# grasingerm/polymer-stats

Hardware: AMD Instinct MI355X
Metric: MC monomer-updates/sec (whole node) at n=100 (higher is better)
Workload: dtype f64

## Files before the change

polymer_stats_amd/csrc/pstat_kernels.hip:

```cpp
#include "pstat_device.h"

#include <hip/hip_runtime.h>
#include <math.h>
#include <type_traits>

#include "../../include/pstat.h"
#include "pstat_math.h"

#ifndef PSTAT_GM_DEPTH
#define PSTAT_GM_DEPTH 2
#endif
#ifndef PSTAT_GI_DEPTH
#define PSTAT_GI_DEPTH 1
#endif
#ifndef PSTAT_GI_CC
#define PSTAT_GI_CC 1
#endif
#ifndef PSTAT_UNROLL_ISING
#define PSTAT_UNROLL_ISING 16
#endif
#ifndef PSTAT_UNROLL
#define PSTAT_UNROLL 16
#endif

namespace pstat {

#ifndef PSTAT_PART

template <typename R, typename G>
__global__ void init_kernel(SweepArgs A, DevState S, const CaseConst *__restrict__ cases,
                            int chain_type, int energy_type, double phi_step, double theta_step,
                            InitOpts io) {
  int64_t c = (int64_t)blockIdx.x * blockDim.x + threadIdx.x;
  if (c >= S.C) return;
  const int64_t icase = c / A.chains_per_case, local = c % A.chains_per_case;
  const CaseConst cc = cases[icase];
  R *th = (R *)S.ang, *ph = (R *)S.ang + A.n * S.C;
  G g;
  g.seed(cc.seed, cc.chain_id0 + (uint64_t)local);
  if (io.use_x0 == 2) {
    for (int64_t i = 0; i < A.n; ++i)
      ph[i * S.C + c] = store_phi_rad<R>(io.x0_vec[2 * i] + io.dx0_phi * u01<double>(g.next()));
    for (int64_t i = 0; i < A.n; ++i)
      th[i * S.C + c] = store_theta_rad<R>(io.x0_vec[2 * i + 1] + io.dx0_theta * u01<double>(g.next()));
  } else if (io.use_x0) {
    for (int64_t i = 0; i < A.n; ++i)
      ph[i * S.C + c] = store_phi_rad<R>(io.x0_phi + io.dx0_phi * u01<double>(g.next()));
    for (int64_t i = 0; i < A.n; ++i)
      th[i * S.C + c] = store_theta_rad<R>(io.x0_theta + io.dx0_theta * u01<double>(g.next()));
  } else {
    for (int64_t i = 0; i < A.n; ++i) ph[i * S.C + c] = store_phi<R>(u01<double>(g.next()));
    for (int64_t i = 0; i < A.n; ++i) th[i * S.C + c] = store_theta<R>(u01<double>(g.next()));
  }

  double r[3] = {0, 0, 0}, p[3] = {0, 0, 0}, usum = 0, upair = 0, omega = 0, c2sum = 0, psisum = 0;
  double pnx = 0, pny = 0, pnz = 0, pmx = 0, pmy = 0, pmz = 0;
  for (int64_t i = 0; i < A.n; ++i) {
    double t = load_theta<R>(th[i * S.C + c]), f = load_phi<R>(ph[i * S.C + c]);
    double st = sin(t), ct = cos(t), sp = sin(f), cp = cos(f);
    double nx = cp * st, ny = sp * st, nz = ct, mx, my, mz;
    if (chain_type == PSTAT_DIELECTRIC)
      dipole<double, PSTAT_DIELECTRIC>((cc.K1 - cc.K2) * cc.E0, cc.K2 * cc.E0, nx, ny, nz, mx, my, mz);
    else
      dipole<double, PSTAT_POLAR>(cc.mu, 0.0, nx, ny, nz, mx, my, mz);
    r[0] += cc.b * nx; r[1] += cc.b * ny; r[2] += cc.b * nz;
    p[0] += mx; p[1] += my; p[2] += mz;
    usum += -0.5 * cc.E0 * mz;
    omega += log(st);
    c2sum += ct * ct;
    if (i > 0) {
      const double psi = acos(fmin(1.0, fmax(-1.0, pnx * nx + pny * ny + pnz * nz)));
      psisum += psi;
      usum += cc.kappa / 2 * (psi - cc.psi0) * (psi - cc.psi0);
    }
    if (energy_type == PSTAT_ISING && i > 0) {
      double h = -cc.b / 2;
      upair += pair_term<double>(h * (pnx + nx), h * (pny + ny), h * (pnz + nz), pmx, pmy, pmz, mx, my, mz);
    }
    pnx = nx; pny = ny; pnz = nz; pmx = mx; pmy = my; pmz = mz;
  }
  double U = usum + upair - (r[0] * cc.Fx + r[2] * cc.Fz);
  S.obs[OBS_R1 * S.C + c] = r[0]; S.obs[OBS_R2 * S.C + c] = r[1]; S.obs[OBS_R3 * S.C + c] = r[2];
  S.obs[OBS_P1 * S.C + c] = p[0]; S.obs[OBS_P2 * S.C + c] = p[1]; S.obs[OBS_P3 * S.C + c] = p[2];
  S.obs[OBS_U * S.C + c] = U; S.obs[OBS_USUM * S.C + c] = usum;
  S.obs[OBS_C2 * S.C + c] = c2sum; S.obs[OBS_PSI * S.C + c] = psisum;
  g.store(S.rng + c, S.C);
  S.stepsz[0 * S.C + c] = phi_step; S.stepsz[1 * S.C + c] = theta_step;
  S.win[0 * S.C + c] = 0; S.win[1 * S.C + c] = 0;
  S.nacc_total[c] = 0;
  for (int q = 0; q < NSUMS; ++q) S.sums[q * S.C + c] = 0.0;
  S.wnorm[c] = 0.0;
  S.lag[c] = 0.0;
  S.uref[c] = usum;
  S.nanrej[c] = 0;
  (void)omega;
}

#endif


struct Draw {
  uint32_t idx, cell, wphi, wth, weps, wflip;
  uint32_t w0;
};

template <typename G, bool WIDE> struct StepGen : G {};
template <> struct StepGen<Mwc64x, true> {
  uint64_t t;
  uint32_t sh;
  __device__ inline void load(const uint32_t *p, int64_t stride) {
    t = (uint64_t)p[0] | ((uint64_t)p[stride] << 32);
    sh = 32;
    asm volatile("" : "+v"(sh));
  }
  __device__ inline uint32_t next() {
    const uint32_t x = (uint32_t)t, r = x ^ (uint32_t)(t >> 32);
    t = (uint64_t)x * Mwc64x::A + (t >> sh);
    return r;
  }
  __device__ inline void store(uint32_t *p, int64_t stride) const {
    p[0] = (uint32_t)t; p[stride] = (uint32_t)(t >> 32); p[2 * stride] = 0u; p[3 * stride] = 0u;
  }
};

template <bool RARE, typename G>
__device__ __forceinline__ Draw draw_step(G &g, uint32_t n, bool flips, uint32_t row_bytes, uint32_t lane_bytes) {
  Draw d;
  d.w0 = g.next();
  d.idx = __umulhi(d.w0, n);
  d.cell = __umul24(d.idx, row_bytes) + lane_bytes;
  d.wphi = g.next();
  d.wflip = 0;
  if constexpr (RARE) {
    if (flips) d.wflip = g.next();
  }
  d.wth = g.next();
  d.weps = g.next();
  return d;
}

template <typename R, typename G, int CT, int EN, bool FX, bool RARE, int ST>
__device__ __forceinline__ void run_segment(const SweepArgs &A, const DevState &S, const CaseConst &cc,
                                            const SweepRare rare, unsigned char *smem, const int lane,
                                            const int64_t c, int64_t step, int64_t remaining, const int blk) {
  using R2 = typename Vec2<R>::type;
  using AG = Ang<R>;
  constexpr bool Q = ST == 1;
  constexpr bool GM = ST == 2;
  static_assert(!Q || sizeof(R) == 4, "the lattice state runs on f32 arithmetic");
  static_assert(!GM || sizeof(R) == 8, "global-memory state: f64");
  constexpr bool GI = GM && EN == PSTAT_ISING;
  constexpr int DEPTH = GI ? PSTAT_GI_DEPTH : PSTAT_GM_DEPTH;
  using Cell = typename std::conditional<Q, uint32_t, R2>::type;
  const int lanes = GM ? 64 : A.lanes;
  unsigned char *const cells = GM ? reinterpret_cast<unsigned char *>(S.work) + (size_t)blk * (size_t)A.n * 64 * sizeof(Cell) : smem;
  Cell *ang = reinterpret_cast<Cell *>(cells);
  const int64_t C = S.C;
  const int n = (int)A.n;

  const R Fz = (R)cc.Fz, Fx = (R)cc.Fx, b = (R)cc.b, kT = (R)cc.kT;
  const R a_or_mu = (CT == PSTAT_DIELECTRIC) ? (R)((cc.K1 - cc.K2) * cc.E0) : (R)cc.mu;
  const R k2e = (R)(cc.K2 * cc.E0);
  const R mhalfE0 = (R)(-0.5 * cc.E0);
  const R hb = (R)(-cc.b / 2);
  const R ising_scale = cc.b == 0.0 ? (R)__builtin_nan("") : (R)(0.0795774715459476679 / fabs(cc.b * cc.b * cc.b / 8));
  const R nbeta_log2e = (R)(-1.4426950408889634 / cc.kT);
  const double ninv_kT = -1.0 / cc.kT;
  (void)ninv_kT;
  (void)Fx; (void)kT; (void)hb; (void)nbeta_log2e; (void)ising_scale;

  R maxphi = 0;
  (void)maxphi;
  if constexpr (Q) {
    const uint16_t *gth = (const uint16_t *)S.ang, *gph = (const uint16_t *)S.ang + (int64_t)n * C;
#pragma unroll 8
    for (int i = 0; i < n; ++i)
      ang[i * lanes + lane] = (uint32_t)gth[(int64_t)i * C + c] | ((uint32_t)gph[(int64_t)i * C + c] << 16);
  } else {
    const R *gth = (const R *)S.ang, *gph = (const R *)S.ang + (int64_t)n * C;
#pragma unroll 8
    for (int i = 0; i < n; ++i) {
      R2 v;
      v.x = gth[(int64_t)i * C + c];
      v.y = gph[(int64_t)i * C + c];
      if constexpr (sizeof(R) == 8) maxphi = fmax(maxphi, fabs(v.y));
      if (GM && i < A.lds_rows) reinterpret_cast<Cell *>(smem)[i * lanes + lane] = v;
      else if constexpr (GM) *reinterpret_cast<Cell *>(cells + ((EN == PSTAT_ISING && PSTAT_GI_CC) ? (uint32_t)lane * (uint32_t)n * (uint32_t)sizeof(Cell) + (uint32_t)i * (uint32_t)sizeof(Cell)
                                                                                                          : (uint32_t)(i * lanes + lane) * (uint32_t)sizeof(Cell))) = v;
      else ang[i * lanes + lane] = v;
    }
  }
  constexpr double th_unit = Q ? 3.14159265358979323846 / 65536.0 : AG::unit;
  constexpr double ph_unit = Q ? 6.28318530717958647692 / 65536.0 : AG::unit;
  StepGen<G, GM> g;
  g.load(S.rng + c, C);
  double phistep_d = S.stepsz[0 * C + c], thstep_d = S.stepsz[1 * C + c];
  R phistep = (R)(phistep_d / ph_unit), thstep = (R)(thstep_d / th_unit);
  int64_t nacc_off = S.win[0 * C + c], natt_off = S.win[1 * C + c];
  int nacc_seg = 0, steps_seg = 0;
  int nnan_seg = 0;
  R O[8];
  O[0] = (R)S.obs[OBS_R1 * C + c]; O[1] = (R)S.obs[OBS_R2 * C + c]; O[2] = (R)S.obs[OBS_R3 * C + c];
  O[3] = (R)S.obs[OBS_P1 * C + c]; O[4] = (R)S.obs[OBS_P2 * C + c]; O[5] = (R)S.obs[OBS_P3 * C + c];
  O[6] = (R)S.obs[OBS_U * C + c]; O[7] = 0;
  R usum = (R)S.obs[OBS_USUM * C + c];
  R lag = RARE ? (R)S.lag[c] : (R)0;
  const bool umb = RARE && rare.umb;
  const R wscale = umb ? (R)((0.2 + 0.8 * exp(-(cc.Fx * cc.Fx + cc.Fz * cc.Fz) / cc.kT)) / cc.kT) : (R)0;
  R uref = umb ? (R)S.uref[c] : (R)0;
  bool regauged = false;
  double wnorm = umb ? S.wnorm[c] : 0.0;
  double sums[NSUMS_BASE];
#pragma unroll
  for (int q = 0; q < NSUMS_BASE; ++q) sums[q] = S.sums[q * C + c];

  const int64_t spa = A.steps_per_adjust;
  int64_t to_adj = A.adaptive ? spa - (step % spa) : 0;
  constexpr int FLUSH = 128;
  const bool flips = RARE && rare.flips;

  using P = typename V2<R>::type;
  const uint32_t row_bytes = (uint32_t)lanes * (uint32_t)sizeof(Cell), lane_bytes = (uint32_t)lane * (uint32_t)sizeof(Cell);
  auto slot = [&](uint32_t off) __attribute__((always_inline)) -> Cell & { return *reinterpret_cast<Cell *>(cells + off); };
  constexpr bool CC = GI && PSTAT_GI_CC;
  const uint32_t chain_g = (uint32_t)lane * (uint32_t)n * (uint32_t)sizeof(Cell);
  auto gofs = [&](const uint32_t idx) __attribute__((always_inline)) -> uint32_t {
    return CC ? chain_g + idx * (uint32_t)sizeof(Cell) : idx * row_bytes + lane_bytes;
  };
  typedef int v4i __attribute__((ext_vector_type(4)));
  struct RowG { Cell l; v4i g; };
  struct RowG3 { RowG c, lo, hi; };
  using Row = typename std::conditional<GI, RowG3, typename std::conditional<GM, RowG, Cell>::type>::type;
  constexpr bool AS = GM && !CC;
  constexpr uint32_t NOWHERE = 0xFFFFFFFFu;
  const uint32_t nL = GM ? (uint32_t)A.lds_rows : 0u;
  const uint32_t trash = nL * row_bytes + lane_bytes;
  const uint32_t gbase = AS ? nL * row_bytes : 0u;
  __amdgpu_buffer_rsrc_t rsrc = __builtin_amdgcn_make_buffer_rsrc(GM ? (void *)(cells + gbase) : (void *)nullptr, 0,
                                                                  GM ? (int)((uint32_t)n * row_bytes - gbase) : 0, 0x00020000);
  auto rdcell = [&](const uint32_t idx, const uint32_t cell) __attribute__((always_inline)) -> RowG {
    RowG r;
    if constexpr (AS) {
      r.l = *reinterpret_cast<Cell *>(smem + (cell < trash ? cell : trash));
      r.g = __builtin_amdgcn_raw_buffer_load_b128(rsrc, cell - gbase, 0, 0);
    } else {
      const bool inL = idx < nL;
      r.l = *reinterpret_cast<Cell *>(smem + (inL ? cell : trash));
      r.g = __builtin_amdgcn_raw_buffer_load_b128(rsrc, inL ? 0xFFFFFFFFu : gofs(idx), 0, 0);
    }
    return r;
  };
  auto resolve = [&](const RowG &r, const uint32_t idx, const uint32_t cell, const Cell &f1, const uint32_t at1,
                     const Cell &f2, const uint32_t at2, const Cell &f3, const uint32_t at3) __attribute__((always_inline)) -> Cell {
    if constexpr (GM) {
      typedef double v2dd __attribute__((ext_vector_type(2)));
      const v2dd gv = __builtin_bit_cast(v2dd, r.g);
      const bool inL = idx < nL;
      Cell a;
      a.x = inL ? r.l.x : gv.x; a.y = inL ? r.l.y : gv.y;
      if constexpr (DEPTH == 3) {
        const bool s3 = at3 == cell;
        a.x = s3 ? f3.x : a.x; a.y = s3 ? f3.y : a.y;
      }
      if constexpr (DEPTH >= 2) {
        const bool s2 = at2 == cell;
        a.x = s2 ? f2.x : a.x; a.y = s2 ? f2.y : a.y;
      }
      const bool s1 = at1 == cell;
      a.x = s1 ? f1.x : a.x; a.y = s1 ? f1.y : a.y;
      return a;
    } else {
      return r.l;
    }
  };
  auto rdrow = [&](const Draw &d) __attribute__((always_inline)) -> Row {
    if constexpr (GI) {
      const bool hasLo = d.idx > 0, hasHi = d.idx + 1 < (uint32_t)n;
      RowG3 r;
      r.c = rdcell(d.idx, d.cell);
      r.lo = rdcell(hasLo ? d.idx - 1 : d.idx, hasLo ? d.cell - row_bytes : d.cell);
      r.hi = rdcell(hasHi ? d.idx + 1 : d.idx, hasHi ? d.cell + row_bytes : d.cell);
      return r;
    } else if constexpr (GM) {
      return rdcell(d.idx, d.cell);
    } else {
      return slot(d.cell);
    }
  };
  auto wr = [&](const Draw &d, const Cell v, const bool ok) __attribute__((always_inline)) {
    if constexpr (AS) {
      const uint32_t at = ok ? d.cell : NOWHERE;
      *reinterpret_cast<Cell *>(smem + (at < trash ? at : trash)) = v;
      typedef double v2dd __attribute__((ext_vector_type(2)));
      const v2dd vv = {v.x, v.y};
      __builtin_amdgcn_raw_buffer_store_b128(__builtin_bit_cast(v4i, vv), rsrc, at - gbase, 0, 0);
    } else if constexpr (GM) {
      const bool inL = d.idx < nL;
      *reinterpret_cast<Cell *>(smem + ((ok && inL) ? d.cell : trash)) = v;
      typedef double v2dd __attribute__((ext_vector_type(2)));
      const v2dd vv = {v.x, v.y};
      __builtin_amdgcn_raw_buffer_store_b128(__builtin_bit_cast(v4i, vv), rsrc, (ok && !inL) ? gofs(d.idx) : 0xFFFFFFFFu, 0, 0);
    } else {
      slot(d.cell) = v;
    }
  };
  Draw dA = draw_step<RARE>(g, (uint32_t)n, flips, row_bytes, lane_bytes), dB = dA;
  Row aA = rdrow(dA), aB = aA;
  Draw dC = dA;
  Row aC = aA;
  Draw dD = dA;
  Row aD = aA;
  Cell fw1_cell{}, fw2_cell{}, fw3_cell{};
  uint32_t fw1_at = ~0u, fw2_at = ~0u, fw3_at = ~0u;
  (void)dC; (void)aC; (void)dD; (void)aD; (void)fw1_cell; (void)fw2_cell; (void)fw3_cell; (void)fw1_at; (void)fw2_at; (void)fw3_at;
  if constexpr (GM && DEPTH >= 2) {
    if (remaining > 1) {
      dB = draw_step<RARE>(g, (uint32_t)n, flips, row_bytes, lane_bytes);
      aB = rdrow(dB);
    }
    if constexpr (DEPTH == 3) {
      if (remaining > 2) {
        dC = draw_step<RARE>(g, (uint32_t)n, flips, row_bytes, lane_bytes);
        aC = rdrow(dC);
      }
    }
  }
  R phistep3 = 3 * phistep, thstep3 = 3 * thstep;
  (void)phistep3; (void)thstep3;
  P stepv = {thstep, phistep}, step3v = {thstep3, phistep3};
  (void)stepv; (void)step3v;
  int left = (int)remaining;
  P Orxy = {O[0], O[1]}, Opxy = {O[3], O[4]};
  P Oz = {O[2], O[5]};
  R OU = O[6];
  const P bb = {b, b};
  (void)bb;

  auto refresh_totals = [&]() {
    double tx = 0, ty = 0, tz = 0, qx = 0, qy = 0, qz = 0, tu = 0, tp = 0;
    R pnx = 0, pny = 0, pnz = 0, pmx = 0, pmy = 0, pmz = 0;
#pragma unroll 1
    for (int i = 0; i < n; ++i) {
      const Cell a = ang[i * lanes + lane];
      R thi, phi;
      if constexpr (Q) { thi = q16_theta_turns(a & 0xFFFFu); phi = q16_phi_turns(a >> 16); }
      else { thi = a.x; phi = a.y; }
      R si, ci, spi, cpi, mix, miy, miz;
      AG::sc(thi, &si, &ci);
      AG::sc(phi, &spi, &cpi);
      const R nix = cpi * si, niy = spi * si, niz = ci;
      dipole<R, CT>(a_or_mu, k2e, nix, niy, niz, mix, miy, miz);
      tx += (double)nix; ty += (double)niy; tz += (double)niz;
      qx += (double)mix; qy += (double)miy; qz += (double)miz;
      tu += (double)(mhalfE0 * miz);
      if constexpr (EN == PSTAT_ISING) {
        if (i > 0)
          tp += (double)pair_term_fast(hb * (pnx + nix), hb * (pny + niy), hb * (pnz + niz), pmx, pmy, pmz, mix, miy, miz);
        pnx = nix; pny = niy; pnz = niz; pmx = mix; pmy = miy; pmz = miz;
      }
    }
    auto opaque = [](R v) __attribute__((always_inline)) -> R { asm volatile("" : "+v"(v)); return v; };
    const double bd = (double)b;
    Orxy.x = opaque((R)tx); Orxy.y = opaque((R)ty); Oz.x = opaque((R)tz);
    Opxy.x = opaque((R)qx); Opxy.y = opaque((R)qy); Oz.y = opaque((R)qz);
    usum = opaque((R)tu);
    OU = opaque((R)(tu + tp - ((double)Fx * bd * tx + (double)Fz * bd * tz)));
  };

  if constexpr (sizeof(R) == 4) refresh_totals();

  auto run_steps = [&](auto fold_tag) __attribute__((always_inline)) {
  constexpr bool FOLD = decltype(fold_tag)::value;
  while (left > 0) {
    int chunk = left < FLUSH ? left : FLUSH;
    if (A.adaptive && to_adj < chunk) chunk = (int)to_adj;
    P a1rxy = {0, 0}, a1pxy = {0, 0}, a2rxy = {0, 0}, a2pxy = {0, 0};
    P a1z = {0, 0}, a2z = {0, 0};
    R a1U = 0, a2U = 0;
    R accw = 0;

    auto one_step = [&](const Draw &d, const Row &a0_, Draw &dn, Row &an, const bool more)
        __attribute__((always_inline)) {
      Cell a0, aLo{}, aHi{};
      (void)aLo; (void)aHi;
      if constexpr (GI) {
        const bool hasLo = d.idx > 0, hasHi = d.idx + 1 < (uint32_t)n;
        a0 = resolve(a0_.c, d.idx, d.cell, fw1_cell, fw1_at, fw2_cell, fw2_at, fw3_cell, fw3_at);
        aLo = resolve(a0_.lo, hasLo ? d.idx - 1 : d.idx, hasLo ? d.cell - row_bytes : d.cell, fw1_cell, fw1_at, fw2_cell, fw2_at, fw3_cell, fw3_at);
        aHi = resolve(a0_.hi, hasHi ? d.idx + 1 : d.idx, hasHi ? d.cell + row_bytes : d.cell, fw1_cell, fw1_at, fw2_cell, fw2_at, fw3_cell, fw3_at);
      } else if constexpr (GM) {
        a0 = resolve(a0_, d.idx, d.cell, fw1_cell, fw1_at, fw2_cell, fw2_at, fw3_cell, fw3_at);
      } else {
        a0 = a0_;
      }
      if (more) {
        dn = draw_step<RARE>(g, (uint32_t)n, flips, row_bytes, lane_bytes);
        an = rdrow(dn);
        __builtin_amdgcn_sched_barrier(0);
      }
      R eps;
      if constexpr (sizeof(R) == 8) eps = 0;
      else eps = bits12(d.weps);
      (void)eps;
      R th0, ph0, th1, ph1;
      bool inside = true;
      uint32_t cell1 = 0;
      if constexpr (Q) {
        uint32_t k0 = a0 & 0xFFFFu;
        const uint32_t j0 = a0 >> 16;
        th0 = q16_theta_turns(k0);
        ph0 = q16_phi_turns(j0);
        if constexpr (RARE) {
          if (flips && (d.wflip >> 31)) k0 = 65535u - k0;
        }
        const int k1 = (int)k0 + q16_disp(thstep, sym11<R>(d.wth));
        const uint32_t j1 = (j0 + (uint32_t)q16_disp(phistep, sym11<R>(d.wphi))) & 0xFFFFu;
        inside = (uint32_t)k1 < 65536u;
        const uint32_t k1c = (uint32_t)min(max(k1, 0), 65535);
        th1 = q16_theta_turns(k1c);
        ph1 = q16_phi_turns(j1);
        cell1 = k1c | (j1 << 16);
      } else {
        th0 = a0.x; ph0 = a0.y;
        R flip = 0;
        if constexpr (RARE) {
          if (flips && (d.wflip >> 31)) flip = AG::theta_max - 2 * th0;
        }
        if constexpr (sizeof(R) == 8) {
          auto rounded = [](R v) __attribute__((always_inline)) -> R { asm volatile("" : "+v"(v)); return v; };
          const R dphi = rounded(phistep * rounded(sym11<R>(d.wphi)));
          R dth = rounded(thstep * rounded(sym11<R>(d.wth)));
          if constexpr (RARE) dth = rounded(flip + dth);
          ph1 = AG::wrap(ph0 + dphi);
          th1 = fmin(AG::theta_max, fmax((R)0, th0 + dth));
        } else {
          R base = th0;
          if constexpr (RARE) base = th0 + flip;
          const P basev = {base, ph0}, fv = {bits24(d.wth), bits24(d.wphi)};
          const P raw = pfma(stepv, fv, basev - step3v);
          th1 = fmin(AG::theta_max, fmax((R)0, raw.x));
          ph1 = AG::wrap(raw.y);
        }
      }
      R st0, ct0, sp0, cp0, st1, ct1, sp1, cp1;
      AG::sc_theta(th0, &st0, &ct0);
      AG::sc_theta(th1, &st1, &ct1);
      AG::template sc_phi<FOLD>(ph0, &sp0, &cp0);
      AG::template sc_phi<FOLD>(ph1, &sp1, &cp1);
      P dNxy, dMxy, D;
      R dpair = 0;
      if constexpr (EN == PSTAT_ISING && sizeof(R) == 4) {
        const P S01 = {st0, st1}, X01 = P{cp0, cp1} * S01, Y01 = P{sp0, sp1} * S01, C01 = {ct0, ct1};
        P MX01, MY01, MZ01;
        if constexpr (CT == PSTAT_DIELECTRIC) {
          const P q01 = C01 * P{a_or_mu, a_or_mu};
          MX01 = q01 * X01; MY01 = q01 * Y01;
          MZ01 = pfma(q01, C01, P{k2e, k2e});
        } else {
          const P mus = {a_or_mu, a_or_mu};
          MX01 = mus * X01; MY01 = mus * Y01; MZ01 = mus * C01;
        }
        dNxy = P{X01.y - X01.x, Y01.y - Y01.x};
        dMxy = P{MX01.y - MX01.x, MY01.y - MY01.x};
        D = P{C01.y - C01.x, MZ01.y - MZ01.x};
        P e01 = {0, 0};
        const P m3 = {-3.0f, -3.0f};
#pragma unroll
        for (int side = -1; side <= 1; side += 2) {
          const int j = (int)d.idx + side;
          if (j >= 0 && j < n) {
            const Cell aj = ang[j * lanes + lane];
            R thj, phj;
            if constexpr (Q) { thj = q16_theta_turns(aj & 0xFFFFu); phj = q16_phi_turns(aj >> 16); }
            else { thj = aj.x; phj = aj.y; }
            R sj, cj, spj, cpj, mjx, mjy, mjz;
            AG::sc(thj, &sj, &cj);
            AG::sc(phj, &spj, &cpj);
            const R njx = cpj * sj, njy = spj * sj, njz = cj;
            dipole<R, CT>(a_or_mu, k2e, njx, njy, njz, mjx, mjy, mjz);
            const P rx = X01 + P{njx, njx}, ry = Y01 + P{njy, njy}, rz = C01 + P{njz, njz};
            const P jx = {mjx, mjx}, jy = {mjy, mjy}, jz = {mjz, mjz};
            const P r2 = pfma(rz, rz, pfma(ry, ry, rx * rx));
            const P ir = {__builtin_amdgcn_rsqf(r2.x), __builtin_amdgcn_rsqf(r2.y)};
            const P ir2 = ir * ir;
            const P mimj = pfma(MZ01, jz, pfma(MY01, jy, MX01 * jx));
            const P mir = pfma(MZ01, rz, pfma(MY01, ry, MX01 * rx));
            const P mjr = pfma(jz, rz, pfma(jy, ry, jx * rx));
            const P num = pfma(m3 * ir2, mir * mjr, mimj);
            e01 = pfma(num, ir2 * ir, e01);
          }
        }
        dpair = (e01.y - e01.x) * ising_scale;
      } else {
        const P cs0 = {cp0, sp0}, cs1 = {cp1, sp1};
        const P s0s = {st0, st0}, s1s = {st1, st1};
        const P Nxy0 = cs0 * s0s, Nxy1 = cs1 * s1s;
        P Mxy0, Mxy1;
        R mz0, mz1;
        if constexpr (CT == PSTAT_DIELECTRIC) {
          const R q0 = a_or_mu * ct0, q1 = a_or_mu * ct1;
          const P q0s = {q0, q0}, q1s = {q1, q1};
          Mxy0 = q0s * Nxy0; Mxy1 = q1s * Nxy1;
          mz0 = q0 * ct0 + k2e; mz1 = q1 * ct1 + k2e;
        } else {
          const P mus = {a_or_mu, a_or_mu};
          Mxy0 = mus * Nxy0; Mxy1 = mus * Nxy1;
          mz0 = a_or_mu * ct0; mz1 = a_or_mu * ct1;
        }
        dNxy = Nxy1 - Nxy0; dMxy = Mxy1 - Mxy0;
        const P Z0 = {ct0, mz0}, Z1 = {ct1, mz1};
        D = Z1 - Z0;

        if constexpr (GI) {
          R e0 = 0, e1 = 0;
#pragma unroll
          for (int side = 0; side < 2; ++side) {
            const Cell aj = side ? aHi : aLo;
            const bool has = side ? d.idx + 1 < (uint32_t)n : d.idx > 0;
            R sj, cj, spj, cpj, mjx, mjy, mjz;
            AG::sc_theta(aj.x, &sj, &cj);
            AG::template sc_phi<FOLD>(aj.y, &spj, &cpj);
            const R njx = cpj * sj, njy = spj * sj, njz = cj;
            dipole<R, CT>(a_or_mu, k2e, njx, njy, njz, mjx, mjy, mjz);
            const R t0 = pair_term_fast(hb * (Nxy0.x + njx), hb * (Nxy0.y + njy), hb * (ct0 + njz),
                                        Mxy0.x, Mxy0.y, mz0, mjx, mjy, mjz);
            const R t1 = pair_term_fast(hb * (Nxy1.x + njx), hb * (Nxy1.y + njy), hb * (ct1 + njz),
                                        Mxy1.x, Mxy1.y, mz1, mjx, mjy, mjz);
            e0 += has ? t0 : (R)0; e1 += has ? t1 : (R)0;
          }
          dpair = e1 - e0;
        } else if constexpr (EN == PSTAT_ISING) {
          R e0 = 0, e1 = 0;
  #pragma unroll
          for (int side = -1; side <= 1; side += 2) {
            const int j = (int)d.idx + side;
            if (j >= 0 && j < n) {
              const Cell aj = ang[j * lanes + lane];
              R thj, phj;
              if constexpr (Q) { thj = q16_theta_turns(aj & 0xFFFFu); phj = q16_phi_turns(aj >> 16); }
              else { thj = aj.x; phj = aj.y; }
              R sj, cj, spj, cpj, mjx, mjy, mjz;
              AG::sc(thj, &sj, &cj);
              AG::sc(phj, &spj, &cpj);
              const R njx = cpj * sj, njy = spj * sj, njz = cj;
              dipole<R, CT>(a_or_mu, k2e, njx, njy, njz, mjx, mjy, mjz);
              e0 += pair_term_fast(hb * (Nxy0.x + njx), hb * (Nxy0.y + njy), hb * (ct0 + njz),
                                   Mxy0.x, Mxy0.y, mz0, mjx, mjy, mjz);
              e1 += pair_term_fast(hb * (Nxy1.x + njx), hb * (Nxy1.y + njy), hb * (ct1 + njz),
                                   Mxy1.x, Mxy1.y, mz1, mjx, mjy, mjz);
            }
          }
          dpair = e1 - e0;
        }
      }
      const R dmz = D.y;
      (void)dmz;

      const P dd = D * P{b, mhalfE0};
      const R drz = dd.x, du = dd.y;
      R dUi = du;
      if constexpr (EN == PSTAT_ISING) dUi = du + dpair;
      R dU;
      if constexpr (FX) dU = dUi - (Fx * (b * dNxy.x) + Fz * drz);
      else              dU = dUi - (Fz * drz);

      bool ok;
      R dw = 0;
      if constexpr (RARE) dw = du * wscale;
      if constexpr (sizeof(R) == 8) {
        ok = metropolis_f64(dU, kT, ninv_kT, st1, st0, dw - lag, A.wide_eps != 0, d.weps, d.w0, d.wphi, d.wth);
      } else {
        R e;
        if constexpr (RARE) e = __builtin_amdgcn_exp2f((R)1.44269504f * (dw - lag) + dU * nbeta_log2e);
        else                e = __builtin_amdgcn_exp2f(dU * nbeta_log2e);
        ok = eps * st0 < fma_r(st1, e, st0);
        if constexpr (Q) ok = ok && inside;
      }

      Cell a1;
      if constexpr (Q) a1 = ok ? cell1 : a0;
      else { a1.x = ok ? th1 : th0; a1.y = ok ? ph1 : ph0; }
      if constexpr (GM) { Cell t1; t1.x = th1; t1.y = ph1; wr(d, t1, ok); }
      else wr(d, a1, ok);
      const R m = ok ? (R)1 : (R)0;
      const P mm = {m, m};
      if constexpr (sizeof(R) == 8) {
        Orxy = pfma(mm, bb * dNxy, Orxy);
        Oz = pfma(mm, P{drz, dmz}, Oz);
      } else {
        Orxy = pfma(mm, dNxy, Orxy);
        Oz = pfma(mm, D, Oz);
      }
      Opxy = pfma(mm, dMxy, Opxy);
      if constexpr (EN == PSTAT_ISING) OU = ok ? OU + dU : OU;
      else                             OU = fma_r(m, dU, OU);
      if constexpr (RARE) {
        usum = fma_r(m, du, usum);
        lag = ok ? (R)0 : lag;
      }
      nacc_seg += ok ? 1 : 0;
      if constexpr (EN == PSTAT_ISING) nnan_seg += not_finite(dU) ? 1 : 0;
      if constexpr (GM) {
        fw3_cell = fw2_cell; fw3_at = fw2_at;
        fw2_cell = fw1_cell; fw2_at = fw1_at;
        fw1_cell.x = th1; fw1_cell.y = ph1; fw1_at = ok ? d.cell : ~0u;
      } else if (more) {
        const bool same = dn.cell == d.cell;
        if constexpr (Q) an = same ? a1 : an;
        else if constexpr (!GM) { an.x = same ? a1.x : an.x; an.y = same ? a1.y : an.y; }
      }

      if (umb) {
        bool raise;
        R wrel = umbrella_logw(usum, uref, wscale, raise);
        if constexpr (RARE) {
          if (__builtin_amdgcn_ballot_w64(raise) != 0) {
            if (raise) {
              const double f = exp_f64(-(double)wrel);
              const R fr = (R)f;
              const P ff = {fr, fr};
              a1rxy *= ff; a1pxy *= ff; a2rxy *= ff; a2pxy *= ff; a1z *= ff; a2z *= ff; a1U *= fr; a2U *= fr; accw *= fr;
#pragma unroll
              for (int q = 0; q < NSUMS_BASE; ++q) sums[q] *= f;
              wnorm *= f;
              uref = usum; regauged = true; wrel = 0;
            }
          }
        }
        const R wgt = exp_r(wrel);
        const P ww = {wgt, wgt};
        accw += wgt;
        a1rxy = pfma(ww, Orxy, a1rxy); a1pxy = pfma(ww, Opxy, a1pxy);
        a2rxy = pfma(ww * Orxy, Orxy, a2rxy); a2pxy = pfma(ww * Opxy, Opxy, a2pxy);
        a1z = pfma(ww, Oz, a1z); a1U = fma_r(wgt, OU, a1U);
        a2z = pfma(ww * Oz, Oz, a2z); a2U = fma_r(wgt * OU, OU, a2U);
      } else {
        a1rxy += Orxy; a1pxy += Opxy;
        a2rxy = pfma(Orxy, Orxy, a2rxy); a2pxy = pfma(Opxy, Opxy, a2pxy);
        a1z += Oz; a1U += OU;
        a2z = pfma(Oz, Oz, a2z); a2U = fma_r(OU, OU, a2U);
      }
    };
    int k = 0;
    constexpr int UNROLL = sizeof(R) == 8 ? 2 : (EN == PSTAT_ISING ? PSTAT_UNROLL_ISING : PSTAT_UNROLL);
    if constexpr (GM) {
      if constexpr (DEPTH == 3) {
        const int lim = chunk < left - 3 ? chunk : left - 3;
        for (; k + 4 <= lim; k += 4) {
          one_step(dA, aA, dD, aD, true);
          one_step(dB, aB, dA, aA, true);
          one_step(dC, aC, dB, aB, true);
          one_step(dD, aD, dC, aC, true);
        }
        for (; k < chunk; ++k) {
          one_step(dA, aA, dD, aD, left - k > 3);
          dA = dB; aA = aB;
          dB = dC; aB = aC;
          dC = dD; aC = aD;
        }
      } else if constexpr (DEPTH == 2) {
        const int lim = chunk < left - 2 ? chunk : left - 2;
        for (; k + 3 <= lim; k += 3) {
          one_step(dA, aA, dC, aC, true);
          one_step(dB, aB, dA, aA, true);
          one_step(dC, aC, dB, aB, true);
        }
        for (; k < chunk; ++k) {
          one_step(dA, aA, dC, aC, left - k > 2);
          dA = dB; aA = aB;
          dB = dC; aB = aC;
        }
      } else {
        const int lim = chunk < left - 1 ? chunk : left - 1;
        for (; k + 2 <= lim; k += 2) {
          one_step(dA, aA, dB, aB, true);
          one_step(dB, aB, dA, aA, true);
        }
        for (; k < chunk; ++k) {
          one_step(dA, aA, dB, aB, left - k > 1);
          dA = dB; aA = aB;
        }
      }
    } else {
    for (; k + (UNROLL - 1) < chunk; k += UNROLL) {
#pragma unroll
      for (int u = 0; u < UNROLL; u += 2) {
        one_step(dA, aA, dB, aB, true);
        one_step(dB, aB, dA, aA, u + 2 < UNROLL || left - k > UNROLL);
      }
    }
    for (; k + 1 < chunk; k += 2) {
      one_step(dA, aA, dB, aB, true);
      one_step(dB, aB, dA, aA, left - k > 2);
    }
    if (k < chunk) {
      one_step(dA, aA, dB, aB, left - k > 1);
      dA = dB; aA = aB;
    }
    }
// ... 374 lines not shown
```

polymer_stats_amd/csrc/pstat_math.h:

```cpp
#pragma once

#include <hip/hip_runtime.h>
#include <math.h>
#include <stdint.h>

#include "../../include/pstat.h"

namespace pstat {


template <typename R> struct Vec2;
template <> struct Vec2<float> { using type = float2; };
template <> struct Vec2<double> { using type = double2; };

template <typename R> struct K;
template <> struct K<double> {
  static constexpr double pi = 3.14159265358979323846;
  static constexpr double half_pi = 1.57079632679489661923;
};

__device__ __forceinline__ double exp_f64(const double x) {
  const double k = rint(x * 1.44269504088896338700e+00);
  const double hi = __builtin_fma(-k, 6.93147180369123816490e-01, x);
  const double r = __builtin_fma(-k, 1.90821492927058770002e-10, hi);
  double p = 1.60590438368216145994e-10;
  p = __builtin_fma(p, r, 2.08767569878680989792e-09);
  p = __builtin_fma(p, r, 2.50521083854417187751e-08);
  p = __builtin_fma(p, r, 2.75573192239858906526e-07);
  p = __builtin_fma(p, r, 2.75573192239858906526e-06);
  p = __builtin_fma(p, r, 2.48015873015873015873e-05);
  p = __builtin_fma(p, r, 1.98412698412698412698e-04);
  p = __builtin_fma(p, r, 1.38888888888888888889e-03);
  p = __builtin_fma(p, r, 8.33333333333333333333e-03);
  p = __builtin_fma(p, r, 4.16666666666666666667e-02);
  p = __builtin_fma(p, r, 1.66666666666666666667e-01);
  p = __builtin_fma(p, r, 5.00000000000000000000e-01);
  const double y = 1.0 + __builtin_fma(p, r * r, r);
  double v = ldexp(y, (int)k);
  v = x < -745.2 ? 0.0 : v;
  v = x > 709.8 ? __builtin_inf() : v;
  return v;
}
__device__ __forceinline__ double log_f64(const double x) {
  int e = __builtin_amdgcn_frexp_exp(x);
  double m = __builtin_amdgcn_frexp_mant(x);
  const bool small = m < 7.07106781186547524401e-01;
  m = small ? m + m : m;
  e = small ? e - 1 : e;
  const double f = m - 1.0, t = 2.0 + f;
  double rc = __builtin_amdgcn_rcp(t);
  rc = __builtin_fma(__builtin_fma(-t, rc, 1.0), rc, rc);
  rc = __builtin_fma(__builtin_fma(-t, rc, 1.0), rc, rc);
  const double s = f * rc, z = s * s, w = z * z;
  const double t1 = w * __builtin_fma(w, __builtin_fma(w, 1.531383769920937332e-01, 2.222219843214978396e-01), 3.999999999940941908e-01);
  const double t2 = z * __builtin_fma(w, __builtin_fma(w, __builtin_fma(w, 1.479819860511658591e-01, 1.818357216161805012e-01),
                                                       2.857142874366239149e-01), 6.666666666666735130e-01);
  const double R = t1 + t2, hfsq = 0.5 * f * f, dk = (double)e;
  double v = dk * 6.93147180369123816490e-01 - ((hfsq - (s * (hfsq + R) + dk * 1.90821492927058770002e-10)) - f);
  v = x == 0.0 ? -__builtin_inf() : v;
  v = x < 0.0 ? __builtin_nan("") : v;
  v = x == __builtin_inf() ? x : v;
  return v;
}

template <typename R>
__device__ __forceinline__ R umbrella_logw(const R usum, const R uref, const R wscale, bool &raise) {
  const R wrel = -(usum - uref) * wscale;
  constexpr R T = sizeof(R) == 4 ? (R)30 : (R)300;
  raise = wrel > T;
  return wrel;
}

__device__ __forceinline__ float exp_r(float x) { return __expf(x); }
__device__ __forceinline__ double exp_r(double x) { return exp_f64(x); }
__device__ __forceinline__ float log_r(float x) { return __logf(x); }
__device__ __forceinline__ double log_r(double x) { return log_f64(x); }
__device__ __forceinline__ float fma_r(float a, float b, float c) { return __builtin_fmaf(a, b, c); }
__device__ __forceinline__ double fma_r(double a, double b, double c) { return a * b + c; }

template <typename R>
__device__ __forceinline__ R u01(uint32_t w) {
  if constexpr (sizeof(R) == 4) return __uint_as_float(0x3F800000u | (w >> 9)) - 1.0f;
  else return (R)(w >> 9) * (R)(1.0 / 8388608.0);
}
__device__ __forceinline__ float bits12(uint32_t w) { return __uint_as_float(__builtin_amdgcn_alignbit(0x7Fu, w, 9)); }
__device__ __forceinline__ float bits24(uint32_t w) { return __uint_as_float(__builtin_amdgcn_alignbit(0x80u, w, 9)); }
template <typename R>
__device__ __forceinline__ R sym11(uint32_t w) {
  if constexpr (sizeof(R) == 4) return __uint_as_float(0x40000000u | (w >> 9)) - 3.0f;
  else return __builtin_fma((R)(w >> 9), (R)(1.0 / 4194304.0), (R)-1);
}

__device__ __forceinline__ double eps_uniform(const bool wide, const uint32_t weps, const uint32_t w0, const uint32_t wphi,
                                              const uint32_t wth) {
  const uint32_t lo = ((wth & 511u) << 12) | ((wphi & 511u) << 3) | (w0 & 7u);
  const double e53 = __builtin_fma((double)weps, 2097152.0, (double)lo) * 0x1p-53;
  const double e23 = (double)(weps >> 9) * (1.0 / 8388608.0);
#ifdef PSTAT_NARROW_EPS
  return e23;
#else
  return wide ? e53 : e23;
#endif
}

template <typename Literal>
__device__ __forceinline__ bool metropolis_filter(const double x, const double num, const double den, const uint32_t weps,
                                                  Literal &&literal) {
  const float t = (float)x;
  const float e = __builtin_amdgcn_exp2f(t * 1.44269504f);
  const float fden = (float)den;
  const float lhs = (__uint_as_float(0x3F800000u | (weps >> 9)) - 1.0f) * fden, rhs = e * (float)num;
  const float lhs_hi = __builtin_fmaf(0x1p-23f, fden, lhs);
  const float m = 2e-6f + 1e-6f * __builtin_fabsf(t);
#ifdef PSTAT_NARROW_EPS
  const bool acc = __builtin_fmaf(lhs, m, lhs) < rhs, rej = lhs > __builtin_fmaf(rhs, m, rhs);
  (void)lhs_hi;
#else
  const bool acc = __builtin_fmaf(lhs_hi, m, lhs_hi) < rhs, rej = lhs > __builtin_fmaf(rhs, m, rhs);
#endif
  bool ok = acc;
  if (__builtin_amdgcn_ballot_w64(!(acc || rej)) != 0) {
    const bool lit = literal();
    ok = (acc || rej) ? acc : lit;
  }
  return ok;
}
__device__ __forceinline__ bool metropolis_f64(const double dU, const double kT, const double ninv_kT, const double st1,
                                               const double st0, const double extra, const bool wide, const uint32_t weps,
                                               const uint32_t w0, const uint32_t wphi, const uint32_t wth) {
  return metropolis_filter(dU * ninv_kT + extra, st1, st0, weps, [&]() -> bool {
    const double delta = -dU / kT + log_f64(st1 / st0) + extra;
    const double eps = eps_uniform(wide, weps, w0, wphi, wth);
    return (delta >= 0) || (eps < exp_f64(delta));
  });
}

template <typename R, int CT>
__device__ __forceinline__ void dipole(R a_or_mu, R k2e, R nx, R ny, R nz, R &mx, R &my, R &mz) {
  if constexpr (CT == PSTAT_DIELECTRIC) {
    R a = a_or_mu * nz;
    mx = a * nx; my = a * ny; mz = a * nz + k2e;
  } else {
    mx = a_or_mu * nx; my = a_or_mu * ny; mz = a_or_mu * nz;
  }
}

template <typename R>
__device__ __forceinline__ R pair_term(R rx, R ry, R rz, R mix, R miy, R miz, R mjx, R mjy, R mjz) {
  R r2 = rx * rx + ry * ry + rz * rz;
  R rmag = sqrt(r2);
  R hx = rx / rmag, hy = ry / rmag, hz = rz / rmag;
  R r3 = r2 * rmag;
  R mimj = mix * mjx + miy * mjy + miz * mjz;
  R mir = mix * hx + miy * hy + miz * hz;
  R mjr = mjx * hx + mjy * hy + mjz * hz;
  return (mimj - 3 * mir * mjr) / ((R)(4.0 * 3.14159265358979323846) * r3);
}

__device__ __forceinline__ float pair_term_fast(float rx, float ry, float rz, float mix, float miy, float miz,
                                                float mjx, float mjy, float mjz) {
  const float r2 = __builtin_fmaf(rz, rz, __builtin_fmaf(ry, ry, rx * rx));
  const float ir = __builtin_amdgcn_rsqf(r2);
  const float ir2 = ir * ir;
  const float mimj = __builtin_fmaf(miz, mjz, __builtin_fmaf(miy, mjy, mix * mjx));
  const float mir = __builtin_fmaf(miz, rz, __builtin_fmaf(miy, ry, mix * rx));
  const float mjr = __builtin_fmaf(mjz, rz, __builtin_fmaf(mjy, ry, mjx * rx));
  const float num = __builtin_fmaf(-3.0f * ir2, mir * mjr, mimj);
  return num * (ir2 * ir) * 0.0795774715459476679f;
}
__device__ __forceinline__ double rsqrt_f64(const double x) {
  const double y = __builtin_amdgcn_rsq(x);
  const double e = __builtin_fma(-(x * y), y, 1.0);
  return __builtin_fma(y * e, __builtin_fma(e, 0.375, 0.5), y);
}
__device__ __forceinline__ double pair_term_fast(double rx, double ry, double rz, double mix, double miy,
                                                 double miz, double mjx, double mjy, double mjz) {
  const double r2 = __builtin_fma(rz, rz, __builtin_fma(ry, ry, rx * rx));
  const double y = rsqrt_f64(r2);
  const double ir2 = y * y;
  const double mimj = __builtin_fma(miz, mjz, __builtin_fma(miy, mjy, mix * mjx));
  const double mir = __builtin_fma(miz, rz, __builtin_fma(miy, ry, mix * rx));
  const double mjr = __builtin_fma(mjz, rz, __builtin_fma(mjy, ry, mjx * rx));
  const double num = __builtin_fma(-3.0 * ir2, mir * mjr, mimj);
  return num * (ir2 * y) * 0.0795774715459476679;
}

template <typename T> __device__ __forceinline__ T store_phi(double u) {
  if constexpr (sizeof(T) == 2) return (T)(uint32_t)(u * 65536.0);
  else if constexpr (sizeof(T) == 4) return (T)u;
  else return (T)(6.28318530717958647692 * u);
}
template <typename T> __device__ __forceinline__ T store_theta(double u) {
  if constexpr (sizeof(T) == 2) return (T)(uint32_t)(u * 65536.0);
  else if constexpr (sizeof(T) == 4) return (T)(0.5 * u);
  else return (T)(3.14159265358979323846 * u);
}
template <typename T> __device__ __forceinline__ T store_phi_rad(double phi) {
  if constexpr (sizeof(T) == 8) return (T)phi;
  double t = phi / 6.28318530717958647692;
  t -= floor(t);
  if constexpr (sizeof(T) == 2) return (T)(uint32_t)fmin(65535.0, t * 65536.0);
  else return (T)t;
}
template <typename T> __device__ __forceinline__ T store_theta_rad(double theta) {
  if constexpr (sizeof(T) == 8) return (T)theta;
  else if constexpr (sizeof(T) == 2) return (T)(uint32_t)fmin(65535.0, fmax(0.0, theta / 3.14159265358979323846 * 65536.0));
  else return (T)(theta / 6.28318530717958647692);
}
template <typename T> __host__ __device__ inline double load_phi(T raw) {
  if constexpr (sizeof(T) == 2) return 6.28318530717958647692 * ((double)raw + 0.5) / 65536.0;
  else if constexpr (sizeof(T) == 4) return 6.28318530717958647692 * (double)raw;
  else return (double)raw;
}
template <typename T> __host__ __device__ inline double load_theta(T raw) {
  if constexpr (sizeof(T) == 2) return 3.14159265358979323846 * ((double)raw + 0.5) / 65536.0;
  else if constexpr (sizeof(T) == 4) return 6.28318530717958647692 * (double)raw;
  else return (double)raw;
}
__device__ __forceinline__ float q16_theta_turns(uint32_t k) {
  return __builtin_fmaf(__uint_as_float(0x4B000001u | (k << 1)), 0x1p-18f, -32.0f);
}
__device__ __forceinline__ float q16_phi_turns(uint32_t j) {
  return __builtin_fmaf(__uint_as_float(0x4B000001u | (j << 1)), 0x1p-17f, -64.0f);
}
__device__ __forceinline__ int q16_disp(float step, float s) {
  return (int)__float_as_uint(__builtin_fmaf(step, s, 12582912.0f)) - 0x4B400000;
}

typedef float v2f __attribute__((ext_vector_type(2)));
typedef double v2d __attribute__((ext_vector_type(2)));
template <typename R> struct V2;
template <> struct V2<float> { using type = v2f; };
template <> struct V2<double> { using type = v2d; };
__device__ __forceinline__ v2f pfma(v2f a, v2f b, v2f c) { return __builtin_elementwise_fma(a, b, c); }
__device__ __forceinline__ v2d pfma(v2d a, v2d b, v2d c) { return a * b + c; }

__device__ __forceinline__ void sincos_f64(double x, double *s, double *c) {
  if (!(fabs(x) < 1.0e5)) {
    const double t = rint(x * 1.59154943091895345609e-01);
    x = __builtin_fma(-t, 2.44929359829470641435e-16, __builtin_fma(-t, 6.28318530717958623200e+00, x));
  }
  const double k = rint(x * 6.36619772367581382433e-01);
  const double r0 = __builtin_fma(-k, 1.57079632679489655800e+00, x);
  const double r = __builtin_fma(-k, 6.12323399573676603587e-17, r0);
  double y = __builtin_fma(-k, 6.12323399573676603587e-17, r0 - r);
  y = __builtin_fma(k, 1.49738490485916983e-33, y);
  const double z = r * r;
  const double S1 = -1.66666666666666324348e-01, S2 = 8.33333333332248946124e-03, S3 = -1.98412698298579493134e-04,
               S4 = 2.75573137070700676789e-06, S5 = -2.50507602534068634195e-08, S6 = 1.58969099521155010221e-10;
  const double v = z * r;
  const double ps = __builtin_fma(z, __builtin_fma(z, __builtin_fma(z, __builtin_fma(z, S6, S5), S4), S3), S2);
  const double ks = r - ((z * (0.5 * y - v * ps) - y) - v * S1);
  const double C1 = 4.16666666666666019037e-02, C2 = -1.38888888888741095749e-03, C3 = 2.48015872894767294178e-05,
               C4 = -2.75573143513906633035e-07, C5 = 2.08757232129817482790e-09, C6 = -1.13596475577881948265e-11;
  const double pc = z * __builtin_fma(z, __builtin_fma(z, __builtin_fma(z, __builtin_fma(z, __builtin_fma(z, C6, C5), C4), C3), C2), C1);
  const double hz = 0.5 * z, w = 1.0 - hz;
  const double kc = w + (((1.0 - w) - hz) + (z * pc - r * y));
  const int q = (int)k & 3;
  const double sa = (q & 1) ? kc : ks, ca = (q & 1) ? ks : kc;
  *s = (q & 2) ? -sa : sa;
  *c = ((q + 1) & 2) ? -ca : ca;
}

#define PSTAT_PHI_FOLD 1.0e9
template <bool BOUNDED, bool FOLD = true>
__device__ __forceinline__ void sincos_fast_f64(double x, double *s, double *c) {
  if constexpr (!BOUNDED && FOLD) {
    if (!(fabs(x) < PSTAT_PHI_FOLD)) {
      const double t = rint(x * 1.59154943091895345609e-01);
      x = __builtin_fma(-t, 2.44929359829470641435e-16, __builtin_fma(-t, 6.28318530717958623200e+00, x));
    }
  }
  const double k = rint(x * 6.36619772367581382433e-01);
  const double r = __builtin_fma(-k, 6.12323399573676603587e-17, __builtin_fma(-k, 1.57079632679489655800e+00, x));
  const double z = r * r;
  const double S1 = -1.66666666666666324348e-01, S2 = 8.33333333332248946124e-03, S3 = -1.98412698298579493134e-04,
               S4 = 2.75573137070700676789e-06, S5 = -2.50507602534068634195e-08, S6 = 1.58969099521155010221e-10;
  const double C1 = 4.16666666666666019037e-02, C2 = -1.38888888888741095749e-03, C3 = 2.48015872894767294178e-05,
               C4 = -2.75573143513906633035e-07, C5 = 2.08757232129817482790e-09, C6 = -1.13596475577881948265e-11;
  const double ps = __builtin_fma(z, __builtin_fma(z, __builtin_fma(z, __builtin_fma(z, __builtin_fma(z, S6, S5), S4), S3), S2), S1);
  const double pc = __builtin_fma(z, __builtin_fma(z, __builtin_fma(z, __builtin_fma(z, __builtin_fma(z, C6, C5), C4), C3), C2), C1);
#ifndef PSTAT_THETA_GENERIC_TAIL
  if constexpr (BOUNDED) {
    const double ks = __builtin_fma(r * z, ps, r);
    const double kc = __builtin_fma(z, __builtin_fma(z, pc, -0.5), 1.0);
    const bool one = k == 1.0, two = k == 2.0;
    const double cq = two ? -kc : kc;
    *s = one ? kc : __builtin_fabs(ks);
    *c = one ? -ks : cq;
    return;
  }
#endif
  const uint32_t q = (uint32_t)(int)k;
  const uint32_t odd = q << 31;
  const uint32_t m_kc = (q >> 1) << 31;
  const uint32_t m_ks = m_kc ^ odd;
  const double rs = __hiloint2double((int)(__double2hiint(r) ^ m_ks), __double2loint(r));
  const double ks = __builtin_fma(rs * z, ps, rs);
  const double kc0 = __builtin_fma(z, __builtin_fma(z, pc, -0.5), 1.0);
  const double kc = __hiloint2double((int)(__double2hiint(kc0) ^ m_kc), __double2loint(kc0));
  const bool swap = (int)odd < 0;
  *s = swap ? kc : ks;
  *c = swap ? ks : kc;
}

__device__ __forceinline__ float acos_r(float x) {
  const float a = fabsf(x);
  float p = -0.0012624911f;
  p = __builtin_fmaf(p, a, 0.0066700901f);
  p = __builtin_fmaf(p, a, -0.0170881256f);
  p = __builtin_fmaf(p, a, 0.0308918810f);
  p = __builtin_fmaf(p, a, -0.0501743046f);
  p = __builtin_fmaf(p, a, 0.0889789874f);
  p = __builtin_fmaf(p, a, -0.2145988016f);
  p = __builtin_fmaf(p, a, 1.5707963050f);
  const float r = __builtin_amdgcn_sqrtf(fmaxf(1.0f - a, 0.0f)) * p;
  return x < 0.0f ? 3.14159265358979f - r : r;
}
__device__ __forceinline__ double acos_r(double x) {
  const double a = fabs(x);
  const bool big = a >= 0.5;
  const double z = big ? __builtin_fma(a, -0.5, 0.5) : a * a;
  double p = 2.87578513674215663354e-02;
  p = __builtin_fma(p, z, -1.48518870712472036977e-02);
  p = __builtin_fma(p, z, 1.74008794426940213707e-02);
  p = __builtin_fma(p, z, 5.45750671864035814818e-03);
  p = __builtin_fma(p, z, 1.03228143501857792808e-02);
  p = __builtin_fma(p, z, 1.14791774151849056834e-02);
  p = __builtin_fma(p, z, 1.39712129735529329289e-02);
  p = __builtin_fma(p, z, 1.73523927208699725588e-02);
  p = __builtin_fma(p, z, 2.23721729421498885526e-02);
  p = __builtin_fma(p, z, 3.03819441385312465076e-02);
  p = __builtin_fma(p, z, 4.46428571463554288434e-02);
  p = __builtin_fma(p, z, 7.49999999999843292020e-02);
  p = __builtin_fma(p, z, 1.66666666666666685170e-01);
  const double zp = z * p;
  const double y = __builtin_amdgcn_rsq(z);
  const double s0 = z * y, h0 = 0.5 * y;
  const double r = __builtin_fma(-s0, h0, 0.5);
  const double s1 = __builtin_fma(s0, r, s0), h1 = __builtin_fma(h0, r, h0);
  double sq = __builtin_fma(__builtin_fma(-s1, s1, z), h1, s1);
  sq = z == 0.0 ? 0.0 : sq;
  const double t = big ? sq : x;
  const double as = __builtin_fma(t, zp, t);
  const double small = 1.57079632679489661923 - as;
  const double two = as + as;
  const double bigv = x < 0.0 ? 3.14159265358979323846 - two : two;
  return big ? bigv : small;
}

template <typename R> struct Ang;
template <> struct Ang<double> {
  static constexpr double theta_max = 3.14159265358979323846;
  static constexpr double unit = 1.0;
  static __device__ __forceinline__ void sc(double x, double *s, double *c) { sincos_f64(x, s, c); }
  static __device__ __forceinline__ void sc_theta(double x, double *s, double *c) { sincos_fast_f64<true>(x, s, c); }
  template <bool FOLD = true>
  static __device__ __forceinline__ void sc_phi(double x, double *s, double *c) { sincos_fast_f64<false, FOLD>(x, s, c); }
  static __device__ __forceinline__ double wrap(double x) { return x; }
};
template <> struct Ang<float> {
  static constexpr float theta_max = 0.5f;
  static constexpr double unit = 6.28318530717958647692;
  static __device__ __forceinline__ void sc(float x, float *s, float *c) {
    *s = __builtin_amdgcn_sinf(x);
    *c = __builtin_amdgcn_cosf(x);
  }
  static __device__ __forceinline__ void sc_theta(float x, float *s, float *c) { sc(x, s, c); }
  template <bool FOLD = true>
  static __device__ __forceinline__ void sc_phi(float x, float *s, float *c) { sc(x, s, c); }
  static __device__ __forceinline__ float wrap(float x) { return __builtin_amdgcn_fractf(x); }
};


}
```

Baseline: 102.3 billion.

## Use direct LDS address-space accesses, prime LDS pipeline, branchless theta sincos select

Folds the LDS base address into the per-lane cell offsets so shared-memory reads and writes go through address_space(3) pointers directly, avoiding per-access base additions. For the AS depth-2 path it changes the prologue to issue dummy writes that prime the pipeline. The Metropolis filter now builds the undecided mask from separate ballots of acc and rej. The bounded theta sincos quadrant select is rewritten as integer bit manipulation with bitop3 instead of double compares and selects. These are several unrelated micro-optimisations aimed at cutting instruction count in the hot MC step, with some risk of subtle correctness issues in the bit tricks and address arithmetic.

```diff
diff --git a/polymer_stats_amd/csrc/pstat_kernels.hip b/polymer_stats_amd/csrc/pstat_kernels.hip
--- a/polymer_stats_amd/csrc/pstat_kernels.hip
+++ b/polymer_stats_amd/csrc/pstat_kernels.hip
@@ -233,15 +233,20 @@
   using Row = typename std::conditional<GI, RowG3, typename std::conditional<GM, RowG, Cell>::type>::type;
   constexpr bool AS = GM && !CC;
   constexpr uint32_t NOWHERE = 0xFFFFFFFFu;
+  typedef double v2dd __attribute__((ext_vector_type(2)));
+  typedef __attribute__((address_space(3))) v2dd LdsCell;
+  const uint32_t lds0 = AS ? (uint32_t)(uintptr_t)(__attribute__((address_space(3))) unsigned char *)smem : 0u;
+  const uint32_t lane_cell = lane_bytes + lds0;
   const uint32_t nL = GM ? (uint32_t)A.lds_rows : 0u;
-  const uint32_t trash = nL * row_bytes + lane_bytes;
-  const uint32_t gbase = AS ? nL * row_bytes : 0u;
-  __amdgpu_buffer_rsrc_t rsrc = __builtin_amdgcn_make_buffer_rsrc(GM ? (void *)(cells + gbase) : (void *)nullptr, 0,
-                                                                  GM ? (int)((uint32_t)n * row_bytes - gbase) : 0, 0x00020000);
+  const uint32_t trash = nL * row_bytes + lane_cell;
+  const uint32_t gbase = AS ? nL * row_bytes + lds0 : 0u;
+  __amdgpu_buffer_rsrc_t rsrc = __builtin_amdgcn_make_buffer_rsrc(GM ? (void *)(cells + (gbase - lds0)) : (void *)nullptr, 0,
+                                                                  GM ? (int)((uint32_t)n * row_bytes - (gbase - lds0)) : 0, 0x00020000);
   auto rdcell = [&](const uint32_t idx, const uint32_t cell) __attribute__((always_inline)) -> RowG {
     RowG r;
     if constexpr (AS) {
-      r.l = *reinterpret_cast<Cell *>(smem + (cell < trash ? cell : trash));
+      const v2dd lv = *(LdsCell *)(uintptr_t)(cell < trash ? cell : trash);
+      r.l.x = lv.x; r.l.y = lv.y;
       r.g = __builtin_amdgcn_raw_buffer_load_b128(rsrc, cell - gbase, 0, 0);
     } else {
       const bool inL = idx < nL;
@@ -253,7 +258,6 @@
   auto resolve = [&](const RowG &r, const uint32_t idx, const uint32_t cell, const Cell &f1, const uint32_t at1,
                      const Cell &f2, const uint32_t at2, const Cell &f3, const uint32_t at3) __attribute__((always_inline)) -> Cell {
     if constexpr (GM) {
-      typedef double v2dd __attribute__((ext_vector_type(2)));
       const v2dd gv = __builtin_bit_cast(v2dd, r.g);
       const bool inL = idx < nL;
       Cell a;
@@ -290,21 +294,19 @@
   auto wr = [&](const Draw &d, const Cell v, const bool ok) __attribute__((always_inline)) {
     if constexpr (AS) {
       const uint32_t at = ok ? d.cell : NOWHERE;
-      *reinterpret_cast<Cell *>(smem + (at < trash ? at : trash)) = v;
-      typedef double v2dd __attribute__((ext_vector_type(2)));
       const v2dd vv = {v.x, v.y};
+      *(LdsCell *)(uintptr_t)(at < trash ? at : trash) = vv;
       __builtin_amdgcn_raw_buffer_store_b128(__builtin_bit_cast(v4i, vv), rsrc, at - gbase, 0, 0);
     } else if constexpr (GM) {
       const bool inL = d.idx < nL;
       *reinterpret_cast<Cell *>(smem + ((ok && inL) ? d.cell : trash)) = v;
-      typedef double v2dd __attribute__((ext_vector_type(2)));
       const v2dd vv = {v.x, v.y};
       __builtin_amdgcn_raw_buffer_store_b128(__builtin_bit_cast(v4i, vv), rsrc, (ok && !inL) ? gofs(d.idx) : 0xFFFFFFFFu, 0, 0);
     } else {
       slot(d.cell) = v;
     }
   };
-  Draw dA = draw_step<RARE>(g, (uint32_t)n, flips, row_bytes, lane_bytes), dB = dA;
+  Draw dA = draw_step<RARE>(g, (uint32_t)n, flips, row_bytes, lane_cell), dB = dA;
   Row aA = rdrow(dA), aB = aA;
   Draw dC = dA;
   Row aC = aA;
@@ -313,14 +315,20 @@
   Cell fw1_cell{}, fw2_cell{}, fw3_cell{};
   uint32_t fw1_at = ~0u, fw2_at = ~0u, fw3_at = ~0u;
   (void)dC; (void)aC; (void)dD; (void)aD; (void)fw1_cell; (void)fw2_cell; (void)fw3_cell; (void)fw1_at; (void)fw2_at; (void)fw3_at;
-  if constexpr (GM && DEPTH >= 2) {
+  if constexpr (AS && DEPTH == 2) {
+    auto nothing = []() __attribute__((always_inline)) -> Cell { R z = 0; asm volatile("" : "+v"(z)); return Cell{z, z}; };
+    wr(dA, nothing(), false);
+    if (remaining > 1) dB = draw_step<RARE>(g, (uint32_t)n, flips, row_bytes, lane_cell);
+    aB = rdrow(dB);
+    wr(dB, nothing(), false);
+  } else if constexpr (GM && DEPTH >= 2) {
     if (remaining > 1) {
-      dB = draw_step<RARE>(g, (uint32_t)n, flips, row_bytes, lane_bytes);
+      dB = draw_step<RARE>(g, (uint32_t)n, flips, row_bytes, lane_cell);
       aB = rdrow(dB);
     }
     if constexpr (DEPTH == 3) {
       if (remaining > 2) {
-        dC = draw_step<RARE>(g, (uint32_t)n, flips, row_bytes, lane_bytes);
+        dC = draw_step<RARE>(g, (uint32_t)n, flips, row_bytes, lane_cell);
         aC = rdrow(dC);
       }
     }
@@ -394,7 +402,7 @@
         a0 = a0_;
       }
       if (more) {
-        dn = draw_step<RARE>(g, (uint32_t)n, flips, row_bytes, lane_bytes);
+        dn = draw_step<RARE>(g, (uint32_t)n, flips, row_bytes, lane_cell);
         an = rdrow(dn);
         __builtin_amdgcn_sched_barrier(0);
       }
diff --git a/polymer_stats_amd/csrc/pstat_math.h b/polymer_stats_amd/csrc/pstat_math.h
--- a/polymer_stats_amd/csrc/pstat_math.h
+++ b/polymer_stats_amd/csrc/pstat_math.h
@@ -119,7 +119,8 @@
   const bool acc = __builtin_fmaf(lhs_hi, m, lhs_hi) < rhs, rej = lhs > __builtin_fmaf(rhs, m, rhs);
 #endif
   bool ok = acc;
-  if (__builtin_amdgcn_ballot_w64(!(acc || rej)) != 0) {
+  const uint64_t decided = __builtin_amdgcn_ballot_w64(acc) | __builtin_amdgcn_ballot_w64(rej);
+  if ((__builtin_amdgcn_ballot_w64(true) & ~decided) != 0) {
     const bool lit = literal();
     ok = (acc || rej) ? acc : lit;
   }
@@ -284,10 +285,16 @@
   if constexpr (BOUNDED) {
     const double ks = __builtin_fma(r * z, ps, r);
     const double kc = __builtin_fma(z, __builtin_fma(z, pc, -0.5), 1.0);
-    const bool one = k == 1.0, two = k == 2.0;
-    const double cq = two ? -kc : kc;
-    *s = one ? kc : __builtin_fabs(ks);
-    *c = one ? -ks : cq;
+    const uint32_t kh = (uint32_t)__double2hiint(k);
+    const uint32_t one = (uint32_t)((int32_t)(kh << 11) >> 31);
+    const uint32_t ksh = (uint32_t)__double2hiint(ks), ksl = (uint32_t)__double2loint(ks);
+    const uint32_t kch = (uint32_t)__double2hiint(kc), kcl = (uint32_t)__double2loint(kc);
+    const uint32_t cqh = (kh << 1) + kch;
+    auto sel = [](uint32_t m, uint32_t a, uint32_t b) __attribute__((always_inline)) -> uint32_t {
+      return (uint32_t)__builtin_amdgcn_bitop3_b32((int)m, (int)a, (int)b, 0xCA);
+    };
+    *s = __hiloint2double((int)sel(one, kch, ksh & 0x7FFFFFFFu), (int)sel(one, kcl, ksl));
+    *c = __hiloint2double((int)sel(one, ksh ^ 0x80000000u, cqh), (int)sel(one, ksl, kcl));
     return;
   }
 #endif
```

Result: no change. 103.3 billion (median of 6 runs) (+0.9%).
